# klindsay28/Newton-Krylov_OOC

Hardware: AMD Instinct MI355X
Metric: GMRES JVPs/sec, py_driver_2d iage (value = value_frozen: products on frozen years, the default; value_reference_semantic: the reference's product, two free-running years, same solver, same run) (higher is better)
Workload: dtype f64

## Files before the change

### newton-krylov_ooc_amd/csrc/nk2d_api.hip

```cpp
#include "nk2d_common.h"
#include "nk2d_build_id.h"

#include <algorithm>
#include <cmath>
#include <cstring>
#include <new>

namespace {

template <typename T>
int dev_alloc(nk2d_ctx* c, T** p, size_t n) {
    NK2D_CHECK(c, hipMalloc((void**)p, sizeof(T) * std::max<size_t>(n, 1)));
    NK2D_CHECK(c, hipMemsetAsync(*p, 0, sizeof(T) * std::max<size_t>(n, 1), nk2d_s(c)));
    return 0;
}

int ensure_stage(nk2d_ctx* c, size_t n) {
    if (n <= c->stage_elems) return 0;
    NK2D_CHECK(c, hipStreamSynchronize(nk2d_s(c)));
    if (c->STAGE) NK2D_CHECK(c, hipFree(c->STAGE));
    if (c->hSTAGE) NK2D_CHECK(c, hipHostFree(c->hSTAGE));
    c->STAGE = c->hSTAGE = nullptr;
    c->stage_elems = 0;
    NK2D_CHECK(c, hipMalloc((void**)&c->STAGE, sizeof(double) * n));
// ... 128 lines not shown
    if (key == "pc_fp32") { c->pc_fp32 = value != 0.0; return 0; }
    if (key == "pc_refine") {
        if (!(value >= 0.0 && value <= 4.0)) return nk2d_fail(c, "nk2d_set_option: pc_refine must be 0 .. 4");
        c->pc_refine = (int)value;
        return 0;
    }
    if (key == "pc_two_ended") {
        if (value != 0.0 && value != 1.0) return nk2d_fail(c, "nk2d_set_option: pc_two_ended is 0 or 1");
        c->pc_two_ended = (int)value;
        return 0;
    }
    if (key == "final_fuse") { c->final_fuse = value != 0.0; return 0; }
    if (key == "year_fences") { c->year_fences = value != 0.0; return 0; }
    if (key == "frozen_persistent") { c->frozen_persistent = value != 0.0; return 0; }
    if (key == "frozen_team") { c->frozen_team = value != 0.0; return 0; }
    if (key == "frozen_coef_lds") { c->frozen_coef_lds = (int)value & 15; return 0; }
    if (key == "frozen_by_column") { c->frozen_by_column = (int)value; return 0; }
    if (key == "frozen_cache_after") { c->frozen_cache_after = (int)value; return 0; }
    if (key == "spec_bias") { c->spec_bias = value > 0.0 ? value : 1.0; return 0; }
    if (key == "stream_years") { c->stream_years = (int)value; c->stream_lost = 0; return 0; }
    if (key == "frozen_tape") {
        if (value != 0.0 && value != 1.0) return nk2d_fail(c, "nk2d_set_option: frozen_tape is 0 or 1");
        c->frozen_tape = (int)value;
        return 0;
    }
    if (key == "stream_hist") {
        if (value != 0.0 && value != 1.0) return nk2d_fail(c, "nk2d_set_option: stream_hist is 0 or 1");
        c->stream_hist = (int)value;
        return 0;
    }
    if (key == "stream_hist_mb") {
// ... 386 lines not shown
    c->frozen_team = 1;
    c->frozen_cache_after = 0;
    c->frozen_cache_pieces = 0;
    c->frozen_cache_piece_mb = 1024.0;
    c->frozen_cache_piece_rows = 0;
    c->frozen_cache_early = 0;
    c->frozen_cache_lean = 0;
    c->frozen_lean_years = 0;
    c->frozen_lean_mem_key = 0;
    c->frozen_forced = 0;
    c->frozen_forced_years = 0;
    c->frozen_phosphorus = 0;
    c->frozen_two_waves_last = 0;
    c->frozen_phosphorus_years = c->frozen_two_waves_years = 0;
    c->frozen_cache_piece_allocs = c->frozen_cache_early_requests = 0;
    c->frozen_coef_lds = 15;
    c->frozen_by_column = 1;
    c->strm = nullptr;
    c->spec_bias = 1.0;
    c->stream_two_waves = std::getenv("NK2D_STREAM_TWO_WAVES") ? std::atoi(std::getenv("NK2D_STREAM_TWO_WAVES")) : 1;
    c->stream_years = 1;
    c->stream_on = 0;
    c->stream_lost = 0;
    c->stream_cmds = c->stream_launches = c->stream_timeouts = c->stream_years_run = 0;
    c->frozen_tape = 0;
    c->tape = nullptr;
    c->tape_rec = c->tape_foreign = 0;
    c->tape_years_run = c->tape_builds = c->tape_timeouts = c->tape_fallbacks = 0;
    c->frozen_wpb = 2;
    c->frozen_alloc_async = 1;
    c->barrier_timeout_ms = 2000.0;
// ... 477 lines not shown
    else if (key == "tape_timeouts") v = c->tape_timeouts;
    else if (key == "tape_fallbacks") v = c->tape_fallbacks;
    else if (key == "tape_bytes") v = nk2d_tape_size(c, 0);
    else if (key == "tape_commands") v = nk2d_tape_size(c, 1);
    else if (key.rfind("stream_prof_", 0) == 0) {
        double pr[12];
        NK2D_TRY(nk2d_stream_profile(c, pr));
        const int i = std::atoi(key.c_str() + 12);
        v = (i >= 0 && i < 12) ? (int64_t)pr[i] : 0;
    }
    else if (key == "frozen_launch_us") v = c->frozen_launch_us;
    else if (key == "frozen_cache_pending") v = nk2d_frozen_cache_pending(c);
    else if (key == "frozen_cache_bytes") v = nk2d_frozen_cache_bytes(c);
    else if (key == "frozen_cache_pieces") v = nk2d_frozen_cache_npieces(c);
    else if (key == "frozen_cache_lean") v = nk2d_frozen_cache_is_lean(c);
    else if (key == "frozen_lean_years") v = c->frozen_lean_years;
    else if (key == "frozen_forced_years") v = c->frozen_forced_years;
    else if (key == "frozen_phosphorus_years") v = c->frozen_phosphorus_years;
    else if (key == "frozen_two_waves_years") v = c->frozen_two_waves_years;
    else if (key == "frozen_cache_piece_allocs") v = nk2d_frozen_cache_piece_allocs(c);
    else if (key == "frozen_cache_early_requests") v = c->frozen_cache_early_requests;
    else if (key == "frozen_fallbacks") v = c->frozen_fallbacks;
    else if (key == "frozen_resumes") v = c->frozen_resumes;
    else if (key == "spec_launches_dropped") v = c->cnt_spec_dropped;
    else if (key == "spec_front_launches_dropped") v = c->cnt_front_dropped;
    else if (key == "err_estimates_queued") v = c->cnt_err_queued;
    else if (key == "err_estimates_dropped") v = c->cnt_err_void;
    else return nk2d_fail(c, "nk2d_get_counter: unknown counter " + key);
    if (out) *out = v;
    return 0;
// ... 328 lines not shown
```

### newton-krylov_ooc_amd/csrc/nk2d_bodies.h

```cpp
#pragma once
#include <atomic>
#include <chrono>
#include <cmath>
#include <cstdio>
#include <cstdlib>
#include <cstring>
#include <mutex>
#include <thread>

#include "nk2d_common.h"
#include "nk2d_hostmath.h"


struct DevP {
    int nz, ny, tc, ncol;
    const double *VV, *KH, *WT, *WB, *DZR, *ZM0, *ZM1, *DM, *DMR, *DYR, *BLDMAX;
    double surf[NK2D_MAX_TRACERS], starget[NK2D_MAX_TRACERS], decay[NK2D_MAX_TRACERS], csrc;
    double atol, rtol;
    double ph_hs, ph_mu, ph_sig, ph_rd, ph_rp, ph_vs;
    const double *LIGHT, *UPR;
    const double *SMSREC, *RESTREC;
    int f_sms, f_restore;
    double f_thres_r;
    size_t np;
// ... 731 lines not shown
__device__ __forceinline__ void w_lds_get(const double* s, int r, int lane, double (&v)[E]) {
#pragma unroll
    for (int e = 0; e < E; ++e) v[e] = s[(r * E + e) * 64 + lane];
}
template <int E>
__device__ __forceinline__ void w_lds_put(double* s, int r, int lane, const double (&v)[E]) {
#pragma unroll
    for (int e = 0; e < E; ++e) s[(r * E + e) * 64 + lane] = v[e];
}

struct LdsSrc {
    const double* coef;
    double* w;
    const double* step;
    const double* piv;
};
template <int E>
__device__ __forceinline__ void col_lds_get(const double* s, int r, int lane, double (&v)[E]) {
#pragma unroll
    for (int e = 0; e < E; ++e) v[e] = s[(r * E + e) * 64 + lane];
}
template <int E, int KIND, int FACTOR, int STAGE, int MP = 0, int FINAL = 0, int CL = 0>
__device__ __forceinline__ void newton_fused_body(const DevP& P, const FusedArgs& A, int task, int lane,
                                                  const FinalArgs* fin = nullptr, const LdsSrc* lds = nullptr) {
    const double* coef_lds = (CL & 1) ? lds->coef : nullptr;
    double* w_lds = (CL & 2) ? lds->w : nullptr;
    (void)coef_lds; (void)w_lds;
    const int tr = task / P.ny, j = task - tr * P.ny;
    const int cs_col = (j > 0) ? task - 1 : task, cn_col = (j < P.ny - 1) ? task + 1 : task;
    double fr[E], fcr[E], fci[E];
    if (STAGE && A.do_stage) {
        ColCoef<E> cf;
        if constexpr (CL & 1) load_coef_lds<E>(coef_lds, lane, cf);
        else load_coef<E>(P, j, lane, cf);
        double y0[E], ys[E], yn[E];
        load_col<E, MP>(A.st.y, task, lane, y0);
        load_col<E, MP>(A.st.y, cs_col, lane, ys);
        load_col<E, MP>(A.st.y, cn_col, lane, yn);
#pragma unroll
        for (int e = 0; e < E; ++e) { fr[e] = 0.0; fcr[e] = 0.0; fci[e] = 0.0; }
#pragma unroll
        for (int i = 0; i < 3; ++i) {
            double c[E], cs[E], cn[E], kv[E], f[E];
            load_col<E, MP>(A.st.z + i * A.st.nv, task, lane, c);
            load_col<E, MP>(A.st.z + i * A.st.nv, cs_col, lane, cs);
            load_col<E, MP>(A.st.z + i * A.st.nv, cn_col, lane, cn);
            if constexpr (CL & 4) col_lds_get<E>(lds->step, i, lane, kv);
            else load_col<E, MP>(A.st.kv[i], j, lane, kv);
#pragma unroll
            for (int e = 0; e < E; ++e) { c[e] = y0[e] + c[e]; cs[e] = ys[e] + cs[e]; cn[e] = yn[e] + cn[e]; }
            tend_col<E, KIND>(P, cf, c, cs, cn, kv, tr, lane, f);
            if constexpr (KIND == 2) forced_sources<E>(P, A.st.kv[i], j, lane, c, f);
            if constexpr (KIND == 1) {
                double u1[E], u2[E], v1[E], v2[E];
                phos_load_others<E>(P, tr, j, lane, A.st.y, u1, u2);
                phos_load_others<E>(P, tr, j, lane, A.st.z + i * A.st.nv, v1, v2);
                phos_add<E>(u1, u2, v1, v2);
                phos_sources<E>(P, tr, j, lane, c, u1, u2, cf.dzr, f);
            }
// ... 149 lines not shown
        double x1[E];
        load_col<E, MP>(A.sw.xr_old, task, lane, x1);
#pragma unroll
        for (int e = 0; e < E; ++e) fr[e] = x1[e] + fr[e];
        load_col<E, MP>(A.sw.xcr_old, task, lane, x1);
#pragma unroll
        for (int e = 0; e < E; ++e) fcr[e] = x1[e] + fcr[e];
        load_col<E, MP>(A.sw.xci_old, task, lane, x1);
#pragma unroll
        for (int e = 0; e < E; ++e) fci[e] = x1[e] + fci[e];
    }
    if (!A.do_update) {
        store_col<E, MP>(A.sw.xr_new, task, lane, fr);
        store_col<E, MP>(A.sw.xcr_new, task, lane, fcr);
        store_col<E, MP>(A.sw.xci_new, task, lane, fci);
        return;
    }
    double yy[E], w0[E], w1[E], w2[E];
    load_col<E, MP>(A.st.y, task, lane, yy);
    if constexpr (CL & 2) {
        w_lds_get<E>(w_lds, 0, lane, w0); w_lds_get<E>(w_lds, 1, lane, w1); w_lds_get<E>(w_lds, 2, lane, w2);
    } else {
        load_col<E>(A.st.w, task, lane, w0);
        load_col<E>(A.st.w + A.st.nv, task, lane, w1);
        load_col<E>(A.st.w + 2 * A.st.nv, task, lane, w2);
    }
    double acc = 0.0;
#pragma unroll
    for (int e = 0; e < E; ++e) {
        const double sc = P.atol + fabs(yy[e]) * P.rtol;
        const double d0 = fr[e] / sc, d1 = fcr[e] / sc, d2 = fci[e] / sc;
        acc += (d0 * d0 + d1 * d1) + d2 * d2;
        w0[e] = w0[e] + fr[e];
        w1[e] = w1[e] + fcr[e];
        w2[e] = w2[e] + fci[e];
    }
    acc = wave_sum(acc);
    if (lane == 0) st_mp<MP>(A.part + task, acc);
    double* wout = const_cast<double*>(A.st.w);
    if constexpr (FINAL) {
        double z0[E], z1[E], z2[E], yn[E];
#pragma unroll
        for (int e = 0; e < E; ++e) {
            z0[e] = (cT[0][0] * w0[e] + cT[0][1] * w1[e]) + cT[0][2] * w2[e];
            z1[e] = (cT[1][0] * w0[e] + cT[1][1] * w1[e]) + cT[1][2] * w2[e];
            z2[e] = (cT[2][0] * w0[e] + cT[2][1] * w1[e]) + cT[2][2] * w2[e];
            yn[e] = yy[e] + z2[e];
        }
        store_col<E, MP>(fin->ynew, task, lane, yn);
        const double xs[3] = {fin->x0, fin->x1, fin->x2};
        double o[3][E];
#pragma unroll
        for (int e = 0; e < E; ++e) {
            double q[3];
#pragma unroll
            for (int cidx = 0; cidx < 3; ++cidx) q[cidx] = (z0[e] * cP[0][cidx] + z1[e] * cP[1][cidx]) + z2[e] * cP[2][cidx];
#pragma unroll
            for (int i = 0; i < 3; ++i) {
                const double p1 = xs[i], p2 = p1 * xs[i], p3 = p2 * xs[i];
                double v = (q[0] * p1 + q[1] * p2) + q[2] * p3;
                v = v + yy[e];
                o[i][e] = v - yn[e];
            }
        }
#pragma unroll
        for (int i = 0; i < 3; ++i) store_col<E, MP>(fin->znext + i * A.st.nv, task, lane, o[i]);
        double wv[E];
#pragma unroll
        for (int r = 0; r < 3; ++r) {
#pragma unroll
            for (int e = 0; e < E; ++e) wv[e] = (cTI[r][0] * o[0][e] + cTI[r][1] * o[1][e]) + cTI[r][2] * o[2][e];
            if constexpr (CL & 2) w_lds_put<E>(w_lds, r, lane, wv);
            else store_col<E>(wout + r * A.st.nv, task, lane, wv);
        }
        return;
    }
    double* zout = A.st.zout;
    if constexpr (CL & 2) {
        w_lds_put<E>(w_lds, 0, lane, w0); w_lds_put<E>(w_lds, 1, lane, w1); w_lds_put<E>(w_lds, 2, lane, w2);
    } else {
        store_col<E>(wout, task, lane, w0);
        store_col<E>(wout + A.st.nv, task, lane, w1);
        store_col<E>(wout + 2 * A.st.nv, task, lane, w2);
    }
    double zz[E];
#pragma unroll
    for (int r = 0; r < 3; ++r) {
#pragma unroll
        for (int e = 0; e < E; ++e) zz[e] = (cT[r][0] * w0[e] + cT[r][1] * w1[e]) + cT[r][2] * w2[e];
        store_col<E, MP>(zout + r * A.st.nv, task, lane, zz);
    }
}


template <int E>
__device__ __forceinline__ void plane_task(const DevP& P, const VmixArgs& V, const JacOut& J, int ptask, int lane) {
    int ti = ptask / P.ny;
    const int j = ptask - ti * P.ny;
    if (J.stage > 0) ti = (ti == 0) ? J.stage : ((ti <= J.stage) ? ti - 1 : ti);
    double kv[E];
    vmix_body_kv<E>(P, V, ti * P.ny + j, lane, kv);
    if (ti == J.stage) jac_core<E, 0>(P, kv, V.out[ti], J.JL, J.JU, J.JS, J.JN, J.JC, nullptr, nullptr, j, lane);
}

template <int E, int WR>
struct TeamLds {
// ... 998 lines not shown
```

### newton-krylov_ooc_amd/csrc/nk2d_common.h

```cpp
#pragma once

#include <hip/hip_runtime.h>
#include <stdint.h>
#include <string>
#include <mutex>
#include <vector>

#include "../../include/nk2d.h"

#define NK2D_WAVE 64
#define NK2D_WAVES_PER_BLOCK 4
#define NK2D_BLOCK (NK2D_WAVE * NK2D_WAVES_PER_BLOCK)
#define NK2D_MAX_E 8
#define NK2D_OWN_REC_CAP 65536
#define NK2D_CKPT_EVERY 128


struct nk2d_ctx {
    nk2d_desc d;
    int nz, ny, tc, E, nzp, ncol, nreg;
    int kind;
    size_t nv;
    size_t np;
    int dev;
// ... 57 lines not shown
    double growth_cap;
    double* PART;
    double* PART2;
    double* STEP_PART;
    size_t step_part_rows;
    double* STEP_NORM;
    int64_t frozen_fallbacks;
    void* frozen_cache;
    int frozen_persistent;
    int frozen_persistent_max_e;
    double frozen_cache_max_gb;
    int64_t frozen_cache_builds, frozen_persistent_years;
    int frozen_team;
    int frozen_wpb;
    int frozen_coef_lds;
    int frozen_by_column;
    int frozen_alloc_async;
    int frozen_cache_after;
    int frozen_cache_pieces;
    double frozen_cache_piece_mb;
    int64_t frozen_cache_piece_rows;
    int frozen_cache_lean;
    int64_t frozen_lean_years;
    uint64_t frozen_lean_mem_key;
    int frozen_forced;
    int64_t frozen_forced_years;
    int frozen_phosphorus;
    int frozen_two_waves_last;
    int64_t frozen_phosphorus_years;
    int64_t frozen_two_waves_years;
// ... 460 lines not shown
```

### newton-krylov_ooc_amd/csrc/nk2d_frozen.hip

```cpp
#include "nk2d_bodies.h"

#include <algorithm>
#include <vector>

__device__ __forceinline__ RowTabs cache_row_tabs(const CachePiecePtrs& C, int i) {
    const int p = i / C.T.rows;
    return piece_row_tabs(C.C, C.T, C.T.base[p], i - p * C.T.rows);
}

template <int E, int PIECES = 0>
__global__ void __launch_bounds__(NK2D_BLOCK) k_cache_planes(DevP P, const CacheRow* __restrict__ rows, typename CacheArgOf<PIECES>::type C, int n) {
    const int lane = threadIdx.x & 63;
    const long long task = (long long)blockIdx.x * (blockDim.x >> 6) + (threadIdx.x >> 6);
    const long long per_row = 4LL * P.ny;
    if (task >= per_row * n) return;
    const int i = (int)(task / per_row), rem = (int)(task - (long long)i * per_row);
    const int slot = rem / P.ny, j = rem - slot * P.ny;
    const CacheRow& R = rows[i];
    if (slot < 3) {
        double kv[E];
        vmix_body_kv<E>(P, R.v, slot * P.ny + j, lane, kv);
    } else {
        double kv[E], up[E], dn[E], so[E], no[E], ce[E];
        vmix_col_regs<E>(P, R.v.bldmin, R.v.y0, R.v.y1, R.v.hw, R.v.frac[3], j, lane, kv);
// ... 50 lines not shown

template <int E, int KIND, int MPX, int FINAL>
__device__ __forceinline__ void frozen_factor_phase(const DevP& P, const FusedArgs& FA, int wave, int lane, const FinalArgs* fin, const LdsSrc* L,
                                                    int coef_lds, bool w_in_lds, double* piv_lds) {
    if (w_in_lds) newton_fused_body<E, KIND, 1, 1, MPX, FINAL, 3>(P, FA, wave, lane, fin, L);
    else if (coef_lds) newton_fused_body<E, KIND, 1, 1, MPX, FINAL, 1>(P, FA, wave, lane, fin, L);
    else newton_fused_body<E, KIND, 1, 1, MPX, FINAL>(P, FA, wave, lane, fin);
    if (piv_lds) {
        asm volatile("s_waitcnt vmcnt(0)" ::: "memory");
        double v[E];
        load_col<E>(FA.sw.fr_inv, wave, lane, v);
        w_lds_put<E>(piv_lds, 0, lane, v);
    }
}

template <int E, int KIND, int TEAM = 0, int PIECES = 0, int LEAN = 0>
__global__ void __launch_bounds__(NK2D_BLOCK) k_frozen_persistent(DevP P, typename FrozenArgOf<PIECES>::type A) {
#include "nk2d_frozen_body.inc"
}
template <int E, int PIECES>
__global__ void __launch_bounds__(NK2D_BLOCK) __attribute__((amdgpu_waves_per_eu(2, 2))) k_frozen_persistent_w2(DevP P, typename FrozenArgOf<PIECES>::type A) {
    constexpr int KIND = 1, TEAM = 0, LEAN = 1;
#include "nk2d_frozen_body.inc"
}

struct nk2d_frozen_cache {
    uint64_t key = 0;
    int64_t n = 0;
    CachePtrs C = {};
    double* slab = nullptr;
// ... 140 lines not shown
        if (fc->alloc_rows) (void)hipFree(fc->alloc_rows);
        if (fc->alloc_frows) (void)hipFree(fc->alloc_frows);
        for (double* p : fc->alloc_pieces) (void)hipFree(p);
    }
    frozen_free_pieces(fc);
    frozen_free_slab(fc);
    if (fc->lean_tab) (void)hipFree(fc->lean_tab);
    if (fc->upr) (void)hipFree(fc->upr);
    delete fc;
    c->frozen_cache = nullptr;
}

static size_t frozen_lds_doubles(int E, int bits, bool by_column, int nwaves) {
    if (!bits) return 0;
    if (!by_column) return (size_t)nwaves * (NK2D_COEF_LDS_DOUBLES(E) + ((bits & 2) ? 3 * E * 64 : 0));
    return NK2D_COEF_LDS_DOUBLES(E) + ((bits & 4) ? 5 * E * 64 : 0) + (size_t)nwaves * (((bits & 2) ? 3 * E * 64 : 0) + ((bits & 8) ? E * 64 : 0));
}

template <class K, class ARGS>
static hipError_t launch_resident(nk2d_ctx* c, K kernel, dim3 grid, dim3 block, DevP& P, ARGS& A, size_t lds_bytes = 0, bool check_only = false) {
    int per_cu = 0;
    hipError_t rc = hipOccupancyMaxActiveBlocksPerMultiprocessor(&per_cu, kernel, (int)block.x, lds_bytes);
    if (rc != hipSuccess) return rc;
    hipDeviceProp_t prop;
    rc = hipGetDeviceProperties(&prop, c->dev);
    if (rc != hipSuccess) return rc;
    if ((long long)per_cu * prop.multiProcessorCount < (long long)grid.x) return hipErrorCooperativeLaunchTooLarge;
    if (check_only) return hipSuccess;
    if (std::getenv("NK2D_DIAG_COOPERATIVE")) {
        void* args[2] = {&P, &A};
        return hipLaunchCooperativeKernel((const void*)kernel, grid, block, args, (unsigned)lds_bytes, nk2d_s(c));
// ... 201 lines not shown
    if (fc->slab || (!fc->pieces.empty() && (fc->piece_rows != B || fc->lean != want_lean || fc->src != want_src))) {
        NK2D_CHECK(c, hipStreamSynchronize(nk2d_s(c)));
        frozen_free_slab(fc);
        frozen_free_pieces(fc);
    }
    if (fc->pieces.size() >= need) return 0;
    size_t free_b = 0, total_b = 0;
    NK2D_CHECK(c, hipMemGetInfo(&free_b, &total_b));
    const double held = 8.0 * (double)fc->pieces.size() * (double)B * (double)per_row;
    if (1.02 * bytes > 0.85 * ((double)free_b + held)) return 0;
    frozen_alloc_pieces_in_thread(fc, c->dev, sizeof(double) * B * per_row, need - fc->pieces.size(), B, want_lean, want_src);
    c->frozen_cache_early_requests++;
    return 0;
}

static int frozen_lds_shape(nk2d_ctx* c, bool phos, int* coef_lds_out, int* by_column_out) {
    int coef_lds = (c->E >= 3) ? c->frozen_coef_lds : 0;
    int by_column = (c->frozen_by_column && c->tc <= NK2D_WAVES_PER_BLOCK && coef_lds &&
                     (c->E >= 5 || (c->frozen_by_column >= 2 && c->E >= 3))) ? 1 : 0;
    if (phos) by_column = 1;
    if (!by_column) coef_lds &= 3;
    hipDeviceProp_t prop;
    NK2D_CHECK(c, hipGetDeviceProperties(&prop, c->dev));
    const int nw = by_column ? c->tc : std::max(1, std::min(NK2D_WAVES_PER_BLOCK, c->frozen_wpb));
    const int wgs = by_column ? c->ny : (c->ncol + nw - 1) / nw;
    const int per_cu = (wgs + prop.multiProcessorCount - 1) / prop.multiProcessorCount;
    for (const int drop : {8, 4, 2}) {
        if (8 * frozen_lds_doubles(c->E, coef_lds, by_column != 0, nw) * (size_t)per_cu <= 160u * 1024u) break;
        coef_lds &= ~drop;
    }
    *coef_lds_out = coef_lds; *by_column_out = by_column;
    return 0;
}

int nk2d_frozen_persistent(nk2d_ctx* c, const double* sched, int64_t n, std::vector<char>* err_rows) {
    if (!frozen_eligible(c, sched, n)) return 1;
    const size_t ntab = (size_t)c->ncol * NK2D_TAB * 64;
    const bool want_pieces = c->frozen_cache_pieces != 0;
    const uint64_t key_full = nk2d_frozen_key(c, sched, n);
    bool want_lean = false;
    NK2D_TRY(frozen_form(c, n, key_full, &want_lean));
    const bool want_src = frozen_thres(c);
    const bool want_phos = c->kind == 1;
    const size_t per_row = frozen_row_doubles(c, want_lean, want_src);
    const size_t B = want_pieces ? frozen_piece_rows(c, want_lean, want_src) : 0, need = want_pieces ? ((size_t)n + B - 1) / B : 0;
    const double bytes = want_pieces ? 8.0 * (double)need * (double)B * (double)per_row : 8.0 * (double)n * (double)per_row;
    if (bytes > c->frozen_cache_max_gb * 1.0e9) return 1;
    if (want_phos) {
        FrozenPieceArgs A0 = {};
        NK2D_TRY(frozen_lds_shape(c, true, &A0.coef_lds, &A0.by_column));
        DevP P0 = make_devp(c);
        const bool has_w2 = c->E >= 5;
        auto fits = [&](bool w2) {
            return want_pieces ? launch_frozen_phos<1>(c, P0, A0, w2, true) : launch_frozen_phos<0>(c, P0, static_cast<FrozenArgs&>(A0), w2, true);
        };
        hipError_t rc = fits(has_w2 && c->frozen_phosphorus == 3);
        if (rc == hipErrorCooperativeLaunchTooLarge && has_w2 && c->frozen_phosphorus == 2) rc = fits(true);
        if (rc == hipErrorCooperativeLaunchTooLarge) { (void)hipGetLastError(); return 1; }
        NK2D_CHECK(c, rc);
    }
    {
        const int st = frozen_adopt(c, (nk2d_frozen_cache*)c->frozen_cache);
        if (st == 1) return 1;
        if (st == 3) { c->frozen_persistent = 0; return 1; }
    }
// ... 249 lines not shown
    A.Y = c->Y; A.YOLD = c->YOLD; A.Z = c->Z; A.ZN = c->ZN; A.W = c->W; A.F = c->F;
    A.BR = c->BR; A.BCR = c->BCR; A.BCI = c->BCI;
    for (int i = 0; i < 2; ++i) { A.XR[i] = c->XR[i]; A.XCR[i] = c->XCR[i]; A.XCI[i] = c->XCI[i]; }
    A.PART = c->YR_PART;
    A.STEP_PART = c->STEP_PART;
    A.rows = fc->frows_dev;
    A.C = fc->C;
    A.n = (int)n;
    A.arrive = (unsigned*)c->YR_SYNC; A.abort_flag = (int*)((char*)c->YR_SYNC + 4096);
    A.out = c->YR_OUT;
    A.spin_ticks = (long long)(c->barrier_timeout_ms * 1.0e5);
    A.fences = c->year_fences;
    A.upr_on = (want_src || want_phos) ? 1 : 0;
    A.SRC = (want_src && !want_pieces) ? fc->C.J + fc->cap_rows * 5 * c->np : nullptr;
    if (want_src || want_phos) P.UPR = fc->upr;
    NK2D_TRY(frozen_lds_shape(c, want_phos, &A.coef_lds, &A.by_column));
    const bool team = c->frozen_team && c->E <= 2;
    const int nblk = team ? c->ncol : nk2d_grid(c->ncol);
    const double* o = c->hYR_OUT;
    {
        A.spin_ticks = (long long)(c->barrier_timeout_ms * 1.0e5);
        hipError_t rc = hipErrorInvalidValue;
        NK2D_CHECK(c, hipMemsetAsync(c->YR_OUT, 0, sizeof(double) * 32, nk2d_s(c)));
        NK2D_CHECK(c, hipEventRecord(c->yr_ev[0], nk2d_s(c)));
        struct Turn {
            int waves;
            explicit Turn(int w) : waves(w) { nk2d_turn_take(waves); }
            ~Turn() { nk2d_turn_give(waves); }
        } turn(team ? 4 * c->ncol : c->ncol);
        c->frozen_two_waves_last = 0;
        if (want_phos) {
// ... 51 lines not shown
```

### newton-krylov_ooc_amd/csrc/nk2d_frozen_body.inc

```
    constexpr int XCD = 0, NB = 1;
    __shared__ int lds_ok;
    __shared__ double team_lds[TEAM ? sizeof(TeamLds<E, 3>) / sizeof(double) : 1];
    constexpr int MPX = XCD ? 2 : 1;
    const int lane = threadIdx.x & 63;
    int wg = (int)blockIdx.x;
    const int tw = uni_i((int)(threadIdx.x >> 6));
    const bool by_col = !TEAM && !XCD && NB != 0 && A.by_column != 0;
    const int wave = TEAM ? uni_i(wg) : (by_col ? uni_i(tw * P.ny + wg) : uni_i(wg * (int)(blockDim.x >> 6) + (int)(threadIdx.x >> 6)));
    const bool col_wave = wave < P.ncol && (!by_col || (tw < P.tc && wg < P.ny));
    int nb_left, nb_right;
    if constexpr (TEAM) {
        const int nb_j = wave % P.ny;
        nb_left = (nb_j > 0) ? wg - 1 : -1;
        nb_right = (nb_j < P.ny - 1) ? wg + 1 : -1;
    } else if (by_col) {
        nb_left = (wg > 0) ? wg - 1 : -1;
        nb_right = (wg < P.ny - 1) ? wg + 1 : -1;
    } else {
        const int wpb = (int)(blockDim.x >> 6);
        const int c0 = wg * wpb, cl = min(c0 + wpb - 1, P.ncol - 1);
        nb_left = (c0 % P.ny > 0) ? wg - 1 : -1;
        nb_right = (cl % P.ny < P.ny - 1) ? wg + 1 : -1;
    }
    NeighbourSync nbs{(unsigned*)((char*)A.arrive + 8192), A.abort_flag, wg, nb_left, nb_right, 0u, &lds_ok, A.spin_ticks, A.fences};
    const size_t nv = A.C.nv;
    int swapY = 0, swapZ = 0, status = 0, done = 0;
    int pc_p = 0, pc_r = 0;
    (void)pc_p; (void)pc_r;
#define FZ_Y (swapY ? A.YOLD : A.Y)
#define FZ_YOLD (swapY ? A.Y : A.YOLD)
#define FZ_Z (swapZ ? A.ZN : A.Z)
#define FZ_ZN (swapZ ? A.Z : A.ZN)
#define FZ_SYNC() \
    if (!nbs.sync()) { status = 1; goto finish; }
    constexpr bool COEF_LDS = NB != 0 && !TEAM && !XCD && E >= 3;
    extern __shared__ double dyn_lds[];
    const bool w_in_lds = COEF_LDS && (A.coef_lds & 2) != 0;
    const bool step_in_lds = COEF_LDS && by_col && (A.coef_lds & 4) != 0;
    const bool piv_in_lds = COEF_LDS && by_col && (A.coef_lds & 8) != 0;
    const int nwv = (int)(blockDim.x >> 6);
    double* my_coef;
    double* my_w;
    double* step_lds = nullptr;
    double* my_piv = nullptr;
    if (by_col) {
        double* p = dyn_lds;
        my_coef = p; p += NK2D_COEF_LDS_DOUBLES(E);
        step_lds = p; p += step_in_lds ? 5 * E * 64 : 0;
        my_w = p + (size_t)tw * (3 * E * 64); p += w_in_lds ? (size_t)nwv * 3 * E * 64 : 0;
        my_piv = p + (size_t)tw * (E * 64);
    } else {
        my_coef = dyn_lds + (size_t)(threadIdx.x >> 6) * (NK2D_COEF_LDS_DOUBLES(E) + (w_in_lds ? 3 * E * 64 : 0));
        my_w = my_coef + NK2D_COEF_LDS_DOUBLES(E);
    }
    const LdsSrc L = {my_coef, my_w, step_lds, my_piv};
    (void)L;
    if constexpr (COEF_LDS) {
        if (A.coef_lds && col_wave && (!by_col || tw == 0)) {
            ColCoef<E> cf;
            load_coef<E>(P, wave % P.ny, lane, cf);
            store_coef_lds<E>(my_coef, lane, cf);
        }
        if (by_col && A.coef_lds) __syncthreads();
    }
    int lds_step = -1;
    (void)lds_step;
    if (col_wave && (!TEAM || tw == 0)) {
        double zero[E];
#pragma unroll
        for (int e = 0; e < E; ++e) zero[e] = 0.0;
#pragma unroll
// ... 68 lines not shown
                    FA.sw.fr_tab = T.fr_tab; FA.sw.fc_tabr = T.fc_tabr; FA.sw.fc_tabi = T.fc_tabi;
                } else {
                    FA.sw.fr_inv = A.C.fr_inv + (size_t)i * nv; FA.sw.fc_invr = A.C.fc_invr + (size_t)i * nv;
                    FA.sw.fc_invi = A.C.fc_invi + (size_t)i * nv;
                    FA.sw.fr_tab = A.C.fr_tab + (size_t)i * A.C.ntab; FA.sw.fc_tabr = A.C.fc_tabr + (size_t)i * A.C.ntab;
                    FA.sw.fc_tabi = A.C.fc_tabi + (size_t)i * A.C.ntab;
                }
                FA.sw.f32 = 0;
                FA.sw.br = A.BR; FA.sw.bcr = A.BCR; FA.sw.bci = A.BCI;
                FA.sw.xr_old = src ? A.XR[1] : A.XR[0]; FA.sw.xcr_old = src ? A.XCR[1] : A.XCR[0];
                FA.sw.xci_old = src ? A.XCI[1] : A.XCI[0];
                FA.sw.xr_new = src ? A.XR[0] : A.XR[1]; FA.sw.xcr_new = src ? A.XCR[0] : A.XCR[1];
                FA.sw.xci_new = src ? A.XCI[0] : A.XCI[1];
                FA.sw.first = first ? 1 : 0;
                FA.part = (k == n_iter - 1) ? A.STEP_PART + (size_t)(3 * i) * P.ncol
                                            : ((k == n_iter - 2) ? A.STEP_PART + (size_t)(3 * i + 1) * P.ncol : A.PART);
                FA.do_stage = do_stage ? 1 : 0; FA.do_update = do_update ? 1 : 0; FA.delta = delta ? 1 : 0;
                if constexpr (COEF_LDS) {
                    if (step_in_lds && lds_step != i) {
                        for (int r = tw; r < 5; r += nwv) {
                            double v[E];
                            const double* src = (r == 0) ? FA.st.kv[0] : ((r == 1) ? FA.st.kv[1] : ((r == 2) ? FA.st.kv[2]
                                                : ((r == 3) ? FA.sw.JL : FA.sw.JU)));
                            load_col<E, MPX>(src, wave % P.ny, lane, v);
                            w_lds_put<E>(step_lds, r, lane, v);
                        }
                        if constexpr (!LEAN) {
                        if (piv_in_lds && col_wave) {
                            double v[E];
                            load_col<E>(FA.sw.fr_inv, wave, lane, v);
                            w_lds_put<E>(my_piv, 0, lane, v);
// ... 12 lines not shown
                    if constexpr (TEAM) {
                        if constexpr (LEAN) {
                            if (col_wave && fac)
                                newton_team_body<E, KIND, 1, 1, 4, 1, MPX>(PK, FA, *reinterpret_cast<TeamLds<E, 3>*>(team_lds), wave, tw, lane, &Fin);
                        }
                        if (col_wave && !fac)
                            newton_team_body<E, KIND, 0, 1, 4, 1, MPX>(P, FA, *reinterpret_cast<TeamLds<E, 3>*>(team_lds), wave, tw, lane, &Fin);
                    } else if (col_wave && fac) {
                        if constexpr (LEAN && COEF_LDS) frozen_factor_phase<E, KIND, MPX, 1>(PK, FA, wave, lane, &Fin, &L, A.coef_lds, w_in_lds, piv_in_lds ? my_piv : nullptr);
                        else if constexpr (LEAN) newton_fused_body<E, KIND, 1, 1, MPX, 1>(PK, FA, wave, lane, &Fin);
                    } else if (col_wave) {
                        bool taken = false;
                        if constexpr (KIND == 0 && E <= 2) {
                            if (m == 1) { newton_single_body<E, MPX, 1>(P, FA, wave, lane, &Fin); taken = true; }
                        }
                        if constexpr (COEF_LDS) {
                            if (step_in_lds && piv_in_lds) { newton_fused_body<E, KIND, 0, 1, MPX, 1, 15>(P, FA, wave, lane, &Fin, &L); taken = true; }
                            else if (step_in_lds) { newton_fused_body<E, KIND, 0, 1, MPX, 1, 7>(P, FA, wave, lane, &Fin, &L); taken = true; }
                            else if (w_in_lds) { newton_fused_body<E, KIND, 0, 1, MPX, 1, 3>(P, FA, wave, lane, &Fin, &L); taken = true; }
                            else if (A.coef_lds) { newton_fused_body<E, KIND, 0, 1, MPX, 1, 1>(P, FA, wave, lane, &Fin, &L); taken = true; }
                        }
                        if (!taken) newton_fused_body<E, KIND, 0, 1, MPX, 1>(P, FA, wave, lane, &Fin);
                    }
                    swapY ^= 1;
                    if (do_stage) swapZ ^= 1;
                } else {
                    if constexpr (TEAM) {
                        if constexpr (LEAN) {
                            if (col_wave && fac)
                                newton_team_body<E, KIND, 1, 1, 4, 0, MPX>(PK, FA, *reinterpret_cast<TeamLds<E, 3>*>(team_lds), wave, tw, lane, nullptr);
                        }
                        if (col_wave && !fac)
                            newton_team_body<E, KIND, 0, 1, 4, 0, MPX>(P, FA, *reinterpret_cast<TeamLds<E, 3>*>(team_lds), wave, tw, lane, nullptr);
                    } else if (col_wave && fac) {
                        if constexpr (LEAN && COEF_LDS) frozen_factor_phase<E, KIND, MPX, 0>(PK, FA, wave, lane, nullptr, &L, A.coef_lds, w_in_lds, piv_in_lds ? my_piv : nullptr);
                        else if constexpr (LEAN) newton_fused_body<E, KIND, 1, 1, MPX, 0>(PK, FA, wave, lane);
                    } else if (col_wave) {
                        bool taken = false;
                        if constexpr (KIND == 0 && E <= 2) {
                            if (m == 1) { newton_single_body<E, MPX, 0>(P, FA, wave, lane); taken = true; }
                        }
                        if constexpr (COEF_LDS) {
                            if (step_in_lds && piv_in_lds) { newton_fused_body<E, KIND, 0, 1, MPX, 0, 15>(P, FA, wave, lane, nullptr, &L); taken = true; }
                            else if (step_in_lds) { newton_fused_body<E, KIND, 0, 1, MPX, 0, 7>(P, FA, wave, lane, nullptr, &L); taken = true; }
                            else if (w_in_lds) { newton_fused_body<E, KIND, 0, 1, MPX, 0, 3>(P, FA, wave, lane, nullptr, &L); taken = true; }
                            else if (A.coef_lds) { newton_fused_body<E, KIND, 0, 1, MPX, 0, 1>(P, FA, wave, lane, nullptr, &L); taken = true; }
                        }
                        if (!taken) newton_fused_body<E, KIND, 0, 1, MPX, 0>(P, FA, wave, lane);
                    }
                    if (do_stage && do_update) swapZ ^= 1;
                }
                src = 1 - src;
                FZ_SYNC()
            }
        }
        if (with_err) {
            if (col_wave && (!TEAM || tw == 0)) {
                ErrArgs EA = {};
                EA.sw.JL = J; EA.sw.JU = J + A.C.np; EA.sw.JS = J + 2 * A.C.np; EA.sw.JN = J + 3 * A.C.np; EA.sw.JC = J + 4 * A.C.np;
                EA.sw.fr_inv = LEAN ? A.C.fr_inv : (PIECES ? T.fr_inv : A.C.fr_inv + (size_t)i * nv);
                EA.sw.fr_tab = LEAN ? A.C.fr_tab : (PIECES ? T.fr_tab : A.C.fr_tab + (size_t)i * A.C.ntab);
                EA.sw.xr_old = A.XR[0]; EA.sw.xr_new = A.XR[1];
                EA.f = A.F; EA.z = FZ_Z; EA.y = FZ_Y; EA.nv = nv; EA.h = R.h;
                EA.part = A.STEP_PART + (size_t)(3 * i + 2) * P.ncol;
                EA.stage = 0; EA.last = 1;
                err_fused_body<E, KIND, MPX>(P, EA, wave, lane);
            }
            FZ_SYNC()
            if (col_wave && (!TEAM || tw == 0)) {
                FinalArgs Fin;
                Fin.ynew = FZ_YOLD;
                Fin.znext = FZ_ZN;
                Fin.x0 = R.x0; Fin.x1 = R.x1; Fin.x2 = R.x2;
                Fin.nblk_cols = 0;
                step_tail_body<E, MPX>(FZ_Y, FZ_Z, nv, Fin, A.W, wave, lane);
                if constexpr (COEF_LDS) {
                    if (w_in_lds) {
                        asm volatile("s_waitcnt vmcnt(0)" ::: "memory");
#pragma unroll
                        for (int r = 0; r < 3; ++r) {
                            double wv[E];
                            load_col<E, (TEAM ? MPX : 0)>(A.W + r * nv, wave, lane, wv);
                            w_lds_put<E>(my_w, r, lane, wv);
                        }
                    }
                }
            }
            swapY ^= 1;
            swapZ ^= 1;
            FZ_SYNC()
// ... 4 lines not shown
    if constexpr (COEF_LDS) {
        if (w_in_lds && col_wave) {
#pragma unroll
            for (int r = 0; r < 3; ++r) {
                double wv[E];
                w_lds_get<E>(my_w, r, lane, wv);
                store_col<E>(A.W + r * nv, wave, lane, wv);
            }
        }
    }
    if (status != 0 && threadIdx.x == 0) A.out[0] = (double)status;
    if (wg == 0 && threadIdx.x == 0) {
        A.out[1] = (double)done; A.out[2] = (double)swapY; A.out[3] = (double)swapZ; A.out[4] = (double)nbs.phase;
    }
#undef FZ_SYNC
#undef FZ_Y
#undef FZ_YOLD
#undef FZ_Z
#undef FZ_ZN
```

Before: 7.951.

## Keep each wave's own-column y and z in LDS/registers across Newton iterations

Adds two new LDS bits (16, 32). With them, a wave's own column of y is cached in LDS and its own z stages are held in registers across Newton iterations of the frozen persistent kernel, so those columns are no longer reloaded from global memory. It also skips the weighted-norm partial-sum reduction on iterations whose result is unused. The cost is extra LDS and register pressure, more template instantiations, and cache validity that must be invalidated correctly on fallback paths.

```diff
diff --git a/newton-krylov_ooc_amd/csrc/nk2d_api.hip b/newton-krylov_ooc_amd/csrc/nk2d_api.hip
--- a/newton-krylov_ooc_amd/csrc/nk2d_api.hip
+++ b/newton-krylov_ooc_amd/csrc/nk2d_api.hip
@@ -166,7 +166,7 @@
     if (key == "year_fences") { c->year_fences = value != 0.0; return 0; }
     if (key == "frozen_persistent") { c->frozen_persistent = value != 0.0; return 0; }
     if (key == "frozen_team") { c->frozen_team = value != 0.0; return 0; }
-    if (key == "frozen_coef_lds") { c->frozen_coef_lds = (int)value & 15; return 0; }
+    if (key == "frozen_coef_lds") { c->frozen_coef_lds = (int)value & 63; return 0; }
     if (key == "frozen_by_column") { c->frozen_by_column = (int)value; return 0; }
     if (key == "frozen_cache_after") { c->frozen_cache_after = (int)value; return 0; }
     if (key == "spec_bias") { c->spec_bias = value > 0.0 ? value : 1.0; return 0; }
@@ -583,7 +583,8 @@
     c->frozen_two_waves_last = 0;
     c->frozen_phosphorus_years = c->frozen_two_waves_years = 0;
     c->frozen_cache_piece_allocs = c->frozen_cache_early_requests = 0;
-    c->frozen_coef_lds = 15;
+    c->frozen_coef_lds = 63;
+    c->frozen_lds_bits = 0;
     c->frozen_by_column = 1;
     c->strm = nullptr;
     c->spec_bias = 1.0;
@@ -1091,6 +1092,7 @@
     else if (key == "frozen_cache_bytes") v = nk2d_frozen_cache_bytes(c);
     else if (key == "frozen_cache_pieces") v = nk2d_frozen_cache_npieces(c);
     else if (key == "frozen_cache_lean") v = nk2d_frozen_cache_is_lean(c);
+    else if (key == "frozen_lds_bits") v = c->frozen_lds_bits;
     else if (key == "frozen_lean_years") v = c->frozen_lean_years;
     else if (key == "frozen_forced_years") v = c->frozen_forced_years;
     else if (key == "frozen_phosphorus_years") v = c->frozen_phosphorus_years;
diff --git a/newton-krylov_ooc_amd/csrc/nk2d_bodies.h b/newton-krylov_ooc_amd/csrc/nk2d_bodies.h
--- a/newton-krylov_ooc_amd/csrc/nk2d_bodies.h
+++ b/newton-krylov_ooc_amd/csrc/nk2d_bodies.h
@@ -769,6 +769,12 @@
     double* w;
     const double* step;
     const double* piv;
+    double* y;
+};
+template <int E>
+struct OwnState {
+    double z[3][E];
+    int valid;
 };
 template <int E>
 __device__ __forceinline__ void col_lds_get(const double* s, int r, int lane, double (&v)[E]) {
@@ -777,7 +783,8 @@
 }
 template <int E, int KIND, int FACTOR, int STAGE, int MP = 0, int FINAL = 0, int CL = 0>
 __device__ __forceinline__ void newton_fused_body(const DevP& P, const FusedArgs& A, int task, int lane,
-                                                  const FinalArgs* fin = nullptr, const LdsSrc* lds = nullptr) {
+                                                  const FinalArgs* fin = nullptr, const LdsSrc* lds = nullptr,
+                                                  OwnState<E>* own = nullptr) {
     const double* coef_lds = (CL & 1) ? lds->coef : nullptr;
     double* w_lds = (CL & 2) ? lds->w : nullptr;
     (void)coef_lds; (void)w_lds;
@@ -789,7 +796,16 @@
         if constexpr (CL & 1) load_coef_lds<E>(coef_lds, lane, cf);
         else load_coef<E>(P, j, lane, cf);
         double y0[E], ys[E], yn[E];
-        load_col<E, MP>(A.st.y, task, lane, y0);
+        if constexpr (CL & 16) {
+            if (!own->valid) {
+                load_col<E, MP>(A.st.y, task, lane, y0);
+                w_lds_put<E>(lds->y, 0, lane, y0);
+            } else {
+                col_lds_get<E>(lds->y, 0, lane, y0);
+            }
+        } else {
+            load_col<E, MP>(A.st.y, task, lane, y0);
+        }
         load_col<E, MP>(A.st.y, cs_col, lane, ys);
         load_col<E, MP>(A.st.y, cn_col, lane, yn);
 #pragma unroll
@@ -797,7 +813,16 @@
 #pragma unroll
         for (int i = 0; i < 3; ++i) {
             double c[E], cs[E], cn[E], kv[E], f[E];
-            load_col<E, MP>(A.st.z + i * A.st.nv, task, lane, c);
+            if constexpr (CL & 32) {
+                if (own->valid) {
+#pragma unroll
+                    for (int e = 0; e < E; ++e) c[e] = own->z[i][e];
+                } else {
+                    load_col<E, MP>(A.st.z + i * A.st.nv, task, lane, c);
+                }
+            } else {
+                load_col<E, MP>(A.st.z + i * A.st.nv, task, lane, c);
+            }
             load_col<E, MP>(A.st.z + i * A.st.nv, cs_col, lane, cs);
             load_col<E, MP>(A.st.z + i * A.st.nv, cn_col, lane, cn);
             if constexpr (CL & 4) col_lds_get<E>(lds->step, i, lane, kv);
@@ -977,10 +1002,22 @@
         store_col<E, MP>(A.sw.xr_new, task, lane, fr);
         store_col<E, MP>(A.sw.xcr_new, task, lane, fcr);
         store_col<E, MP>(A.sw.xci_new, task, lane, fci);
+        if constexpr (CL & 32) {
+#pragma unroll
+            for (int i = 0; i < 3; ++i) {
+#pragma unroll
+                for (int e = 0; e < E; ++e) own->z[i][e] = 0.0;
+            }
+            own->valid = 0;
+        }
         return;
     }
+    const bool norm = A.part != nullptr;
     double yy[E], w0[E], w1[E], w2[E];
-    load_col<E, MP>(A.st.y, task, lane, yy);
+    if (FINAL || norm) {
+        if constexpr (CL & 16) col_lds_get<E>(lds->y, 0, lane, yy);
+        else load_col<E, MP>(A.st.y, task, lane, yy);
+    }
     if constexpr (CL & 2) {
         w_lds_get<E>(w_lds, 0, lane, w0); w_lds_get<E>(w_lds, 1, lane, w1); w_lds_get<E>(w_lds, 2, lane, w2);
     } else {
@@ -988,18 +1025,23 @@
         load_col<E>(A.st.w + A.st.nv, task, lane, w1);
         load_col<E>(A.st.w + 2 * A.st.nv, task, lane, w2);
     }
-    double acc = 0.0;
+    if (norm) {
+        double acc = 0.0;
+#pragma unroll
+        for (int e = 0; e < E; ++e) {
+            const double sc = P.atol + fabs(yy[e]) * P.rtol;
+            const double d0 = fr[e] / sc, d1 = fcr[e] / sc, d2 = fci[e] / sc;
+            acc += (d0 * d0 + d1 * d1) + d2 * d2;
+        }
+        acc = wave_sum(acc);
+        if (lane == 0) st_mp<MP>(A.part + task, acc);
+    }
 #pragma unroll
     for (int e = 0; e < E; ++e) {
-        const double sc = P.atol + fabs(yy[e]) * P.rtol;
-        const double d0 = fr[e] / sc, d1 = fcr[e] / sc, d2 = fci[e] / sc;
-        acc += (d0 * d0 + d1 * d1) + d2 * d2;
         w0[e] = w0[e] + fr[e];
         w1[e] = w1[e] + fcr[e];
         w2[e] = w2[e] + fci[e];
     }
-    acc = wave_sum(acc);
-    if (lane == 0) st_mp<MP>(A.part + task, acc);
     double* wout = const_cast<double*>(A.st.w);
     if constexpr (FINAL) {
         double z0[E], z1[E], z2[E], yn[E];
@@ -1011,6 +1053,7 @@
             yn[e] = yy[e] + z2[e];
         }
         store_col<E, MP>(fin->ynew, task, lane, yn);
+        if constexpr (CL & 16) w_lds_put<E>(lds->y, 0, lane, yn);
         const double xs[3] = {fin->x0, fin->x1, fin->x2};
         double o[3][E];
 #pragma unroll
@@ -1036,6 +1079,14 @@
             if constexpr (CL & 2) w_lds_put<E>(w_lds, r, lane, wv);
             else store_col<E>(wout + r * A.st.nv, task, lane, wv);
         }
+        if constexpr (CL & 32) {
+#pragma unroll
+            for (int i = 0; i < 3; ++i) {
+#pragma unroll
+                for (int e = 0; e < E; ++e) own->z[i][e] = o[i][e];
+            }
+        }
+        if constexpr ((CL & 48) != 0) own->valid = 1;
         return;
     }
     double* zout = A.st.zout;
@@ -1052,7 +1103,12 @@
 #pragma unroll
         for (int e = 0; e < E; ++e) zz[e] = (cT[r][0] * w0[e] + cT[r][1] * w1[e]) + cT[r][2] * w2[e];
         store_col<E, MP>(zout + r * A.st.nv, task, lane, zz);
-    }
+        if constexpr (CL & 32) {
+#pragma unroll
+            for (int e = 0; e < E; ++e) own->z[r][e] = zz[e];
+        }
+    }
+    if constexpr ((CL & 48) != 0) own->valid = 1;
 }
 
 
diff --git a/newton-krylov_ooc_amd/csrc/nk2d_common.h b/newton-krylov_ooc_amd/csrc/nk2d_common.h
--- a/newton-krylov_ooc_amd/csrc/nk2d_common.h
+++ b/newton-krylov_ooc_amd/csrc/nk2d_common.h
@@ -95,6 +95,7 @@
     int frozen_team;
     int frozen_wpb;
     int frozen_coef_lds;
+    int frozen_lds_bits;
     int frozen_by_column;
     int frozen_alloc_async;
     int frozen_cache_after;
diff --git a/newton-krylov_ooc_amd/csrc/nk2d_frozen.hip b/newton-krylov_ooc_amd/csrc/nk2d_frozen.hip
--- a/newton-krylov_ooc_amd/csrc/nk2d_frozen.hip
+++ b/newton-krylov_ooc_amd/csrc/nk2d_frozen.hip
@@ -88,6 +88,7 @@
     }
 }
 
+#define NK2D_FROZEN_OWN(E, KIND, TEAM, LEAN) ((E) >= 5 && (E) <= 7 && ((KIND) == 0 || (KIND) == 2) && !(TEAM) && !(LEAN))
 template <int E, int KIND, int TEAM = 0, int PIECES = 0, int LEAN = 0>
 __global__ void __launch_bounds__(NK2D_BLOCK) k_frozen_persistent(DevP P, typename FrozenArgOf<PIECES>::type A) {
 #include "nk2d_frozen_body.inc"
@@ -258,7 +259,8 @@
 static size_t frozen_lds_doubles(int E, int bits, bool by_column, int nwaves) {
     if (!bits) return 0;
     if (!by_column) return (size_t)nwaves * (NK2D_COEF_LDS_DOUBLES(E) + ((bits & 2) ? 3 * E * 64 : 0));
-    return NK2D_COEF_LDS_DOUBLES(E) + ((bits & 4) ? 5 * E * 64 : 0) + (size_t)nwaves * (((bits & 2) ? 3 * E * 64 : 0) + ((bits & 8) ? E * 64 : 0));
+    return NK2D_COEF_LDS_DOUBLES(E) + ((bits & 4) ? 5 * E * 64 : 0) +
+           (size_t)nwaves * (((bits & 2) ? 3 * E * 64 : 0) + ((bits & 8) ? E * 64 : 0) + ((bits & 16) ? E * 64 : 0));
 }
 
 template <class K, class ARGS>
@@ -490,21 +492,25 @@
     return 0;
 }
 
-static int frozen_lds_shape(nk2d_ctx* c, bool phos, int* coef_lds_out, int* by_column_out) {
+static int frozen_lds_shape(nk2d_ctx* c, bool phos, bool lean, bool pieces, int* coef_lds_out, int* by_column_out) {
     int coef_lds = (c->E >= 3) ? c->frozen_coef_lds : 0;
     int by_column = (c->frozen_by_column && c->tc <= NK2D_WAVES_PER_BLOCK && coef_lds &&
                      (c->E >= 5 || (c->frozen_by_column >= 2 && c->E >= 3))) ? 1 : 0;
     if (phos) by_column = 1;
     if (!by_column) coef_lds &= 3;
+    const bool team = c->frozen_team && c->E <= 2;
+    if (!by_column || phos || (coef_lds & 15) != 15 || !NK2D_FROZEN_OWN(c->E, c->kind, team, lean)) coef_lds &= 15;
     hipDeviceProp_t prop;
     NK2D_CHECK(c, hipGetDeviceProperties(&prop, c->dev));
     const int nw = by_column ? c->tc : std::max(1, std::min(NK2D_WAVES_PER_BLOCK, c->frozen_wpb));
     const int wgs = by_column ? c->ny : (c->ncol + nw - 1) / nw;
     const int per_cu = (wgs + prop.multiProcessorCount - 1) / prop.multiProcessorCount;
-    for (const int drop : {8, 4, 2}) {
+    for (const int drop : {16, 8, 4, 2}) {
         if (8 * frozen_lds_doubles(c->E, coef_lds, by_column != 0, nw) * (size_t)per_cu <= 160u * 1024u) break;
         coef_lds &= ~drop;
     }
+    if ((coef_lds & 15) != 15) coef_lds &= 15;
+    if (pieces && (coef_lds & 48) == 32) coef_lds &= 15;
     *coef_lds_out = coef_lds; *by_column_out = by_column;
     return 0;
 }
@@ -524,7 +530,7 @@
     if (bytes > c->frozen_cache_max_gb * 1.0e9) return 1;
     if (want_phos) {
         FrozenPieceArgs A0 = {};
-        NK2D_TRY(frozen_lds_shape(c, true, &A0.coef_lds, &A0.by_column));
+        NK2D_TRY(frozen_lds_shape(c, true, true, want_pieces, &A0.coef_lds, &A0.by_column));
         DevP P0 = make_devp(c);
         const bool has_w2 = c->E >= 5;
         auto fits = [&](bool w2) {
@@ -804,7 +810,8 @@
     A.upr_on = (want_src || want_phos) ? 1 : 0;
     A.SRC = (want_src && !want_pieces) ? fc->C.J + fc->cap_rows * 5 * c->np : nullptr;
     if (want_src || want_phos) P.UPR = fc->upr;
-    NK2D_TRY(frozen_lds_shape(c, want_phos, &A.coef_lds, &A.by_column));
+    NK2D_TRY(frozen_lds_shape(c, want_phos, want_lean, want_pieces, &A.coef_lds, &A.by_column));
+    c->frozen_lds_bits = A.coef_lds;
     const bool team = c->frozen_team && c->E <= 2;
     const int nblk = team ? c->ncol : nk2d_grid(c->ncol);
     const double* o = c->hYR_OUT;
diff --git a/newton-krylov_ooc_amd/csrc/nk2d_frozen_body.inc b/newton-krylov_ooc_amd/csrc/nk2d_frozen_body.inc
--- a/newton-krylov_ooc_amd/csrc/nk2d_frozen_body.inc
+++ b/newton-krylov_ooc_amd/csrc/nk2d_frozen_body.inc
@@ -33,28 +33,48 @@
 #define FZ_ZN (swapZ ? A.Z : A.ZN)
 #define FZ_SYNC() \
     if (!nbs.sync()) { status = 1; goto finish; }
+#define FZ_OWN_DEAD() \
+    if constexpr (OWN) { \
+        _Pragma("unroll") for (int r_ = 0; r_ < 3; ++r_) { \
+            _Pragma("unroll") for (int e_ = 0; e_ < E; ++e_) own.z[r_][e_] = 0.0; \
+        } \
+    }
     constexpr bool COEF_LDS = NB != 0 && !TEAM && !XCD && E >= 3;
     extern __shared__ double dyn_lds[];
     const bool w_in_lds = COEF_LDS && (A.coef_lds & 2) != 0;
     const bool step_in_lds = COEF_LDS && by_col && (A.coef_lds & 4) != 0;
     const bool piv_in_lds = COEF_LDS && by_col && (A.coef_lds & 8) != 0;
+    constexpr bool OWN = COEF_LDS && NK2D_FROZEN_OWN(E, KIND, TEAM, LEAN);
+    const int own_bits = OWN && by_col ? (A.coef_lds & 48) : 0;
+    (void)own_bits;
     const int nwv = (int)(blockDim.x >> 6);
     double* my_coef;
     double* my_w;
     double* step_lds = nullptr;
     double* my_piv = nullptr;
+    double* my_y = nullptr;
     if (by_col) {
         double* p = dyn_lds;
         my_coef = p; p += NK2D_COEF_LDS_DOUBLES(E);
         step_lds = p; p += step_in_lds ? 5 * E * 64 : 0;
         my_w = p + (size_t)tw * (3 * E * 64); p += w_in_lds ? (size_t)nwv * 3 * E * 64 : 0;
-        my_piv = p + (size_t)tw * (E * 64);
+        my_piv = p + (size_t)tw * (E * 64); p += piv_in_lds ? (size_t)nwv * E * 64 : 0;
+        my_y = p + (size_t)tw * (E * 64);
     } else {
         my_coef = dyn_lds + (size_t)(threadIdx.x >> 6) * (NK2D_COEF_LDS_DOUBLES(E) + (w_in_lds ? 3 * E * 64 : 0));
         my_w = my_coef + NK2D_COEF_LDS_DOUBLES(E);
     }
-    const LdsSrc L = {my_coef, my_w, step_lds, my_piv};
+    const LdsSrc L = {my_coef, my_w, step_lds, my_piv, my_y};
     (void)L;
+    OwnState<OWN ? E : 1> own;
+    own.valid = 0;
+    if constexpr (OWN) {
+#pragma unroll
+        for (int r = 0; r < 3; ++r) {
+#pragma unroll
+            for (int e = 0; e < E; ++e) own.z[r][e] = 0.0;
+        }
+    }
     if constexpr (COEF_LDS) {
         if (A.coef_lds && col_wave && (!by_col || tw == 0)) {
             ColCoef<E> cf;
@@ -153,7 +173,8 @@
                 FA.sw.xci_new = src ? A.XCI[0] : A.XCI[1];
                 FA.sw.first = first ? 1 : 0;
                 FA.part = (k == n_iter - 1) ? A.STEP_PART + (size_t)(3 * i) * P.ncol
-                                            : ((k == n_iter - 2) ? A.STEP_PART + (size_t)(3 * i + 1) * P.ncol : A.PART);
+                                            : ((k == n_iter - 2) ? A.STEP_PART + (size_t)(3 * i + 1) * P.ncol
+                                                                 : ((!TEAM && E >= 3) ? nullptr : A.PART));
                 FA.do_stage = do_stage ? 1 : 0; FA.do_update = do_update ? 1 : 0; FA.delta = delta ? 1 : 0;
                 if constexpr (COEF_LDS) {
                     if (step_in_lds && lds_step != i) {
@@ -196,13 +217,19 @@
                         if constexpr (KIND == 0 && E <= 2) {
                             if (m == 1) { newton_single_body<E, MPX, 1>(P, FA, wave, lane, &Fin); taken = true; }
                         }
+                        if constexpr (OWN) {
+                            if (own_bits == 48) { newton_fused_body<E, KIND, 0, 1, MPX, 1, 63>(P, FA, wave, lane, &Fin, &L, &own); taken = true; }
+                            else if (!PIECES && own_bits == 32) { newton_fused_body<E, KIND, 0, 1, MPX, 1, 47>(P, FA, wave, lane, &Fin, &L, &own); taken = true; }
+                            else if (own_bits == 16) { newton_fused_body<E, KIND, 0, 1, MPX, 1, 31>(P, FA, wave, lane, &Fin, &L, &own); FZ_OWN_DEAD() taken = true; }
+                        }
                         if constexpr (COEF_LDS) {
-                            if (step_in_lds && piv_in_lds) { newton_fused_body<E, KIND, 0, 1, MPX, 1, 15>(P, FA, wave, lane, &Fin, &L); taken = true; }
-                            else if (step_in_lds) { newton_fused_body<E, KIND, 0, 1, MPX, 1, 7>(P, FA, wave, lane, &Fin, &L); taken = true; }
-                            else if (w_in_lds) { newton_fused_body<E, KIND, 0, 1, MPX, 1, 3>(P, FA, wave, lane, &Fin, &L); taken = true; }
-                            else if (A.coef_lds) { newton_fused_body<E, KIND, 0, 1, MPX, 1, 1>(P, FA, wave, lane, &Fin, &L); taken = true; }
-                        }
-                        if (!taken) newton_fused_body<E, KIND, 0, 1, MPX, 1>(P, FA, wave, lane, &Fin);
+                            if (taken) {}
+                            else if (step_in_lds && piv_in_lds) { newton_fused_body<E, KIND, 0, 1, MPX, 1, 15>(P, FA, wave, lane, &Fin, &L); FZ_OWN_DEAD() taken = true; }
+                            else if (step_in_lds) { newton_fused_body<E, KIND, 0, 1, MPX, 1, 7>(P, FA, wave, lane, &Fin, &L); FZ_OWN_DEAD() taken = true; }
+                            else if (w_in_lds) { newton_fused_body<E, KIND, 0, 1, MPX, 1, 3>(P, FA, wave, lane, &Fin, &L); FZ_OWN_DEAD() taken = true; }
+                            else if (A.coef_lds) { newton_fused_body<E, KIND, 0, 1, MPX, 1, 1>(P, FA, wave, lane, &Fin, &L); FZ_OWN_DEAD() taken = true; }
+                        }
+                        if (!taken) { newton_fused_body<E, KIND, 0, 1, MPX, 1>(P, FA, wave, lane, &Fin); FZ_OWN_DEAD() }
                     }
                     swapY ^= 1;
                     if (do_stage) swapZ ^= 1;
@@ -222,13 +249,19 @@
                         if constexpr (KIND == 0 && E <= 2) {
                             if (m == 1) { newton_single_body<E, MPX, 0>(P, FA, wave, lane); taken = true; }
                         }
+                        if constexpr (OWN) {
+                            if (own_bits == 48) { newton_fused_body<E, KIND, 0, 1, MPX, 0, 63>(P, FA, wave, lane, nullptr, &L, &own); taken = true; }
+                            else if (!PIECES && own_bits == 32) { newton_fused_body<E, KIND, 0, 1, MPX, 0, 47>(P, FA, wave, lane, nullptr, &L, &own); taken = true; }
+                            else if (own_bits == 16) { newton_fused_body<E, KIND, 0, 1, MPX, 0, 31>(P, FA, wave, lane, nullptr, &L, &own); FZ_OWN_DEAD() taken = true; }
+                        }
                         if constexpr (COEF_LDS) {
-                            if (step_in_lds && piv_in_lds) { newton_fused_body<E, KIND, 0, 1, MPX, 0, 15>(P, FA, wave, lane, nullptr, &L); taken = true; }
-                            else if (step_in_lds) { newton_fused_body<E, KIND, 0, 1, MPX, 0, 7>(P, FA, wave, lane, nullptr, &L); taken = true; }
-                            else if (w_in_lds) { newton_fused_body<E, KIND, 0, 1, MPX, 0, 3>(P, FA, wave, lane, nullptr, &L); taken = true; }
-                            else if (A.coef_lds) { newton_fused_body<E, KIND, 0, 1, MPX, 0, 1>(P, FA, wave, lane, nullptr, &L); taken = true; }
-                        }
-                        if (!taken) newton_fused_body<E, KIND, 0, 1, MPX, 0>(P, FA, wave, lane);
+                            if (taken) {}
+                            else if (step_in_lds && piv_in_lds) { newton_fused_body<E, KIND, 0, 1, MPX, 0, 15>(P, FA, wave, lane, nullptr, &L); FZ_OWN_DEAD() taken = true; }
+                            else if (step_in_lds) { newton_fused_body<E, KIND, 0, 1, MPX, 0, 7>(P, FA, wave, lane, nullptr, &L); FZ_OWN_DEAD() taken = true; }
+                            else if (w_in_lds) { newton_fused_body<E, KIND, 0, 1, MPX, 0, 3>(P, FA, wave, lane, nullptr, &L); FZ_OWN_DEAD() taken = true; }
+                            else if (A.coef_lds) { newton_fused_body<E, KIND, 0, 1, MPX, 0, 1>(P, FA, wave, lane, nullptr, &L); FZ_OWN_DEAD() taken = true; }
+                        }
+                        if (!taken) { newton_fused_body<E, KIND, 0, 1, MPX, 0>(P, FA, wave, lane); FZ_OWN_DEAD() }
                     }
                     if (do_stage && do_update) swapZ ^= 1;
                 }
@@ -256,6 +289,7 @@
                 Fin.x0 = R.x0; Fin.x1 = R.x1; Fin.x2 = R.x2;
                 Fin.nblk_cols = 0;
                 step_tail_body<E, MPX>(FZ_Y, FZ_Z, nv, Fin, A.W, wave, lane);
+                own.valid = 0;
                 if constexpr (COEF_LDS) {
                     if (w_in_lds) {
                         asm volatile("s_waitcnt vmcnt(0)" ::: "memory");
@@ -290,6 +324,7 @@
         A.out[1] = (double)done; A.out[2] = (double)swapY; A.out[3] = (double)swapZ; A.out[4] = (double)nbs.phase;
     }
 #undef FZ_SYNC
+#undef FZ_OWN_DEAD
 #undef FZ_Y
 #undef FZ_YOLD
 #undef FZ_Z
```

Measured after the change: 8.381, median of 6. +5.4%, better.
